# raphiniert-com/volume_renderer

Hardware: AMD Instinct MI355X
Metric: Mrays/s + achieved HBM GB/s, 1024³ vol @ 1920×1080 HG-shaded, 1/2/4/8 GPU (higher is better)
Workload: dtype f32; 1 GPU; V_shell(1024) fp32 1024^3, 1920x1080, HG 2 lights (example1.m), on-the-fly gradient, rotate(125,25,0) f=3 dist=6 thr=0.9; lights=2, gradient=compute, parallelism=image-column partition x1 (block 16), depth_lanes=2, frames=serial, one HIP stream

## Files before the change

include/vrhip.h:

```cpp
#ifndef VRHIP_H_
#define VRHIP_H_

#include <stddef.h>
#include <stdint.h>

#ifdef __cplusplus
extern "C" {
#endif

enum vr_status {
  VR_OK = 0,
  VR_ERR_ARGUMENT = 1,
  VR_ERR_HANDLE = 2,
  VR_ERR_VRAM = 3,
  VR_ERR_DEVICE = 4,
  VR_ERR_UNSUPPORTED = 5
};

enum vr_location { VR_HOST = 0, VR_DEVICE = 1 };

enum vr_dtype { VR_F32 = 0, VR_U8 = 1, VR_U16 = 2, VR_I16 = 3, VR_F16 = 4 };
#define VR_DTYPE_UNORM 0x100

typedef struct vr_volume {
// ... 95 lines not shown
int vr_render_isosurface_device(vr_context *h, const vr_render_args *args, float level, const vr_partition *part,
                                float *d_out, float *d_depth, float *d_normal,
                                unsigned long long *d_steps , void *stream);

int64_t vr_partition_columns(int64_t w, const vr_partition *part);

int vr_assemble_partitions(const float *d_parts, int64_t w, int64_t h, int32_t block_cols,
                           int32_t num_parts, int64_t max_cols, float *d_out, void *stream);

#define VR_SLAB_PLANES 10
typedef struct vr_slab {
  uint64_t depth;
  uint64_t z_first;
  double z0, z1;
  int32_t direction;
  int32_t reserved;
} vr_slab;
int vr_render_slab(vr_context *h, const vr_render_args *args, const vr_slab *slab, const vr_partition *part,
                   const float *d_state_in, float *d_state_out, void *stream);

int vr_slab_planes(const uint64_t dims[3], const float element_size_um[3], double z0, double z1, uint64_t *first,
                   uint64_t *count);

int vr_depth_lanes(int64_t part_cols, int64_t height);
int vr_depth_lanes_tau(int64_t part_cols, int64_t height, double texels_per_pixel);

int vr_synth_shell_device(float *d_out, uint64_t n, void *stream);

int vr_synth_shell_planes_device(float *d_out, uint64_t n, uint64_t z_first, uint64_t count, void *stream);

int vr_gradient_device(const float *d_data, const uint64_t dims[3], float *d_gx, float *d_gy, float *d_gz,
                       void *stream);


int vr_henyey_greenstein_device(uint32_t n, float g, float *d_out, void *stream);

int vr_normalize_device(const float *d_in, uint64_t n, double new_min, double new_max, float *d_out, void *stream);

int vr_resize_device(const float *d_in, const uint64_t in_dims[3], const uint64_t out_dims[3], float *d_out,
                     void *stream);

int vr_resize_contributions(uint64_t in_len, uint64_t out_len, int32_t *P, double *w, int32_t *idx);

int vr_debug_slot_transition(const int32_t idx_in[3], int32_t sim_em_ab, int32_t sim_em_re,
                             int32_t sim_ab_re, int32_t req_em, int32_t req_ab, int32_t req_re,
                             int32_t idx_out[3], int32_t unbound_out[3]);

const char *vr_last_error(void);

int64_t vr_hip_errors(char *buf, size_t buflen);

int vr_last_march_kernel(char *buf, size_t buflen);

int vr_set_option(const char *name, int64_t value);

const char *vr_version(void);

#ifdef __cplusplus
}
#endif
#endif
```

volume_renderer_amd/_lib.py:

```python
from __future__ import annotations

import ctypes
import os
from ctypes import POINTER, c_char_p, c_float, c_int, c_int32, c_int64, c_size_t, c_uint32, c_uint64, c_void_p

_HERE = os.path.dirname(os.path.abspath(__file__))
_DEFAULT_PATH = os.path.join(_HERE, "libvrhip.so")
LIB_PATH = os.environ.get("VR_LIB_PATH") or _DEFAULT_PATH

VR_OK = 0
VR_HOST = 0
VR_DEVICE = 1
VR_F32, VR_U8, VR_U16, VR_I16, VR_F16 = 0, 1, 2, 3, 4
VR_DTYPE_UNORM = 0x100
VR_PROJ_MIP, VR_PROJ_SUM = 0, 1


class VrVolume(ctypes.Structure):
    _fields_ = [("data", c_void_p), ("dims", c_uint64 * 3), ("last_update", c_uint64),
                ("location", c_int32), ("dtype", c_int32)]


class VrLight(ctypes.Structure):
    _fields_ = [("position", c_float * 3), ("color", c_float * 3)]
# ... 30 lines not shown
        super().__init__(msg)
        self.code = code


_lib = None

SIGNATURES = [
    ("vr_new", c_int, [POINTER(c_void_p)]),
    ("vr_new_multi", c_int, [POINTER(c_int32), c_int32, POINTER(c_void_p)]),
    ("vr_delete", c_int, [c_void_p]),
    ("vr_mem_info", c_int, [c_void_p, c_char_p, c_size_t]),
    ("vr_sync_volumes", c_int, [c_void_p, c_uint64, POINTER(VrVolume), POINTER(VrVolume), POINTER(VrVolume),
                                POINTER(VrVolume), POINTER(VrVolume), POINTER(VrVolume)]),
    ("vr_render", c_int, [c_void_p, POINTER(VrRenderArgs), c_void_p]),
    ("vr_render_stereo", c_int, [c_void_p, POINTER(VrRenderArgs), c_float, c_void_p, c_void_p]),
    ("vr_render_channels", c_int, [POINTER(VrChannel), c_int32, c_int32, c_float, c_void_p]),
    ("vr_render_channels_device", c_int, [POINTER(VrChannel), c_int32, c_int32, c_float, c_void_p, c_void_p]),
    ("vr_sum_channels_device", c_int, [c_void_p, c_int32, c_int32, c_uint64, c_void_p, c_void_p]),
    ("vr_henyey_greenstein", c_int, [c_uint32, c_float, c_void_p]),
    ("vr_timestamp", c_uint64, []),
    ("vr_dtype_size", c_size_t, [c_int32]),
    ("vr_convert_host", c_int, [c_void_p, c_int32, c_uint64, c_void_p]),
    ("vr_render_device", c_int, [c_void_p, POINTER(VrRenderArgs), POINTER(VrPartition), c_void_p, c_void_p,
                                 c_void_p]),
    ("vr_render_stereo_device", c_int, [c_void_p, POINTER(VrRenderArgs), c_float, c_void_p, c_void_p, c_void_p,
                                        c_void_p]),
    ("vr_render_projection", c_int, [c_void_p, POINTER(VrRenderArgs), c_int32, c_void_p, c_void_p]),
    ("vr_render_projection_device", c_int, [c_void_p, POINTER(VrRenderArgs), c_int32, POINTER(VrPartition), c_void_p,
                                            c_void_p, c_void_p, c_void_p]),
    ("vr_render_isosurface", c_int, [c_void_p, POINTER(VrRenderArgs), c_float, c_void_p, c_void_p, c_void_p]),
    ("vr_render_isosurface_device", c_int, [c_void_p, POINTER(VrRenderArgs), c_float, POINTER(VrPartition), c_void_p,
                                            c_void_p, c_void_p, c_void_p, c_void_p]),
    ("vr_partition_columns", c_int64, [c_int64, POINTER(VrPartition)]),
    ("vr_assemble_partitions", c_int, [c_void_p, c_int64, c_int64, c_int32, c_int32, c_int64, c_void_p,
                                       c_void_p]),
    ("vr_depth_lanes", c_int, [c_int64, c_int64]),
    ("vr_depth_lanes_tau", c_int, [c_int64, c_int64, ctypes.c_double]),
    ("vr_render_slab", c_int, [c_void_p, POINTER(VrRenderArgs), POINTER(VrSlab), POINTER(VrPartition), c_void_p,
                                c_void_p, c_void_p]),
    ("vr_slab_planes", c_int, [POINTER(c_uint64), POINTER(c_float), ctypes.c_double, ctypes.c_double,
                               POINTER(c_uint64), POINTER(c_uint64)]),
    ("vr_synth_shell_device", c_int, [c_void_p, c_uint64, c_void_p]),
    ("vr_synth_shell_planes_device", c_int, [c_void_p, c_uint64, c_uint64, c_uint64, c_void_p]),
    ("vr_gradient_device", c_int, [c_void_p, POINTER(c_uint64), c_void_p, c_void_p, c_void_p, c_void_p]),
    ("vr_henyey_greenstein_device", c_int, [c_uint32, c_float, c_void_p, c_void_p]),
    ("vr_normalize_device", c_int, [c_void_p, c_uint64, ctypes.c_double, ctypes.c_double, c_void_p, c_void_p]),
    ("vr_resize_device", c_int, [c_void_p, POINTER(c_uint64), POINTER(c_uint64), c_void_p, c_void_p]),
    ("vr_resize_contributions", c_int, [c_uint64, c_uint64, POINTER(c_int32), c_void_p, c_void_p]),
    ("vr_debug_slot_transition", c_int, [POINTER(c_int32), c_int32, c_int32, c_int32, c_int32, c_int32, c_int32,
                                         POINTER(c_int32), POINTER(c_int32)]),
    ("vr_last_error", c_char_p, []),
    ("vr_hip_errors", c_int64, [c_char_p, c_size_t]),
    ("vr_last_march_kernel", c_int, [c_char_p, c_size_t]),
    ("vr_set_option", c_int, [c_char_p, c_int64]),
    ("vr_version", c_char_p, []),
]


def lib():
    global _lib
    if _lib is None:
        try:
            import torch
        except Exception:
            pass
        if not os.path.exists(LIB_PATH):
            raise ImportError(f"libvrhip.so not built at {LIB_PATH}: run __graft_entry__.build() "
                              "(make -C volume_renderer_amd/csrc)")
        handle = ctypes.CDLL(LIB_PATH)
        for name, res, args in SIGNATURES:
            if LIB_PATH != _DEFAULT_PATH and not hasattr(handle, name):
                continue
            fn = getattr(handle, name)
            fn.restype = res
            fn.argtypes = args
        _lib = handle
    return _lib


def check(rc: int) -> None:
    if rc != VR_OK:
        msg = lib().vr_last_error().decode(errors="replace")
        raise VrError(rc, msg)


def hip_errors() -> tuple[int, list[str]]:
    buf = ctypes.create_string_buffer(32 * 400)
    n = lib().vr_hip_errors(buf, len(buf))
    return int(n), [l for l in buf.value.decode(errors="replace").splitlines() if l]
```

volume_renderer_amd/csrc/vr_capi.hip:

```cpp
#include <hip/hip_runtime.h>

#include <algorithm>
#include <chrono>
#include <cmath>
#include <cstdio>
#include <cstdlib>
#include <cstring>
#include <memory>
#include <mutex>
#include <map>
#include <set>
#include <array>
#include <sstream>
#include <string>
#include <queue>
#include <vector>

#include "../../include/vrhip.h"
#include "vr_device.h"
#include "vr_resources.h"

#ifndef VR_WITH_K8
#define VR_WITH_K8 0
#endif
// ... 824 lines not shown
    slots = cus * 16;
  }
  return slots;
}

#ifndef VR_COUNT_K
#define VR_COUNT_K 0
#endif
#ifndef VR_XCD_RUN
#define VR_XCD_RUN 0
#endif

int depth_lanes(const vr::RenderParams &P) {
  if (const char *ev = test_env("VR_DEPTH_LANES")) {
    const int k = std::atoi(ev);
    if (k == 1 || k == 2 || k == 4 || (k == 8 && VR_WITH_K8)) return k;
  }
  const double waves = std::ceil(P.part_cols / 8.0) * std::ceil(P.height / 8.0);
  const double rounds = waves / device_wave_slots();
  const double tau = P.tau > 0.f ? (double)P.tau : 1.0;
  if (P.lookup) return 4;
  if (rounds < VR_DEPTH_ROUNDS_K2 || tau >= VR_DEPTH_TAU_K4) return 4;
  if (rounds >= VR_DEPTH_ROUNDS_K1 && tau < VR_DEPTH_TAU_K1) return 1;
  return 2;
}

void set_tau_and_slot(vr::RenderParams &P, const vr_render_args *a, double vw) {
  const double f = std::fabs((double)a->props[1]), dist = std::fabs((double)a->props[2]);
  const double tau = (f > 0 && P.width > 0) ? dist * vw / ((double)P.width * f) : 1e30;
  P.tau = (float)std::min(tau, 1e30);
  const int K = P.steps ? 1 : depth_lanes(P);
  P.wide_slot = (tau > 1.5 || (K >= 4 && !P.lookup)) ? 1 : 0;
  if (const char *ev = test_env("VR_WIDE_SLOT")) P.wide_slot = std::atoi(ev) ? 1 : 0;
}

bool short_launch(const vr::RenderParams &P) {
  const double rounds = std::ceil(P.part_cols / 8.0) * std::ceil(P.height / 8.0) * std::max(1, (int)P.views) /
                        device_wave_slots();
  return rounds < VR_SCHED_ROUNDS;
}
#ifndef VR_SCHED_LPT_ROUNDS
#define VR_SCHED_LPT_ROUNDS 32.0
#endif
bool lpt_launch(const vr::RenderParams &P) {
  const double rounds = std::ceil(P.part_cols / 8.0) * std::ceil(P.height / 8.0) * std::max(1, (int)P.views) /
                        device_wave_slots();
  return rounds < VR_SCHED_ROUNDS || rounds >= VR_SCHED_LPT_ROUNDS;
}
bool want_schedule(const vr::RenderParams &P) {
  if (P.views > 2 || (P.views == 2 && test_flag("VR_STEREO_PAIR")) || test_flag_off("VR_SCHED")) return false;
  return test_flag("VR_SCHED") || short_launch(P) || !test_flag_off("VR_SCHED_FULL");
}

uint64_t wg_tail_arg(uint32_t tail_pct) {
  return (uint64_t)tail_pct << 32 | (uint64_t)(device_wave_slots() / 16 * 6);
}

uint64_t frame_key(const vr::RenderParams &P) {
  uint64_t h = 1469598103934665603ull;
  auto mix = [&h](const void *p, size_t n) {
    const unsigned char *c = static_cast<const unsigned char *>(p);
    for (size_t i = 0; i < n; ++i) h = (h ^ c[i]) * 1099511628211ull;
  };
  mix(P.eye, sizeof P.eye);
  mix(P.eye2, sizeof P.eye2);
  mix(P.nx_, sizeof P.nx_);
  mix(P.ydir, sizeof P.ydir);
  mix(P.zdir, sizeof P.zdir);
  mix(&P.focal, sizeof P.focal);
  mix(P.bmin, sizeof P.bmin);
  mix(&P.tstep, sizeof P.tstep);
  mix(&P.thr, sizeof P.thr);
  mix(&P.fa, sizeof P.fa);
  mix(&P.fe, sizeof P.fe);
  mix(&P.em.p, sizeof P.em.p);
  mix(&P.occ, sizeof P.occ);
  const BufPtr &eb = g_tex.bind[g_tex.idx_em];
  const uint64_t ver = (eb && eb->ptr == P.em.p) ? eb->version : 0;
  mix(&ver, sizeof ver);
  return h | 1u;
}

#ifndef VR_PRED_STEP_TEXELS
#define VR_PRED_STEP_TEXELS 8.0
#endif
hipError_t predict_costs(const vr::RenderParams &P, int K, uint32_t nb_view, uint32_t *cost, hipStream_t stream) {
  const int TW = K == 1 ? 8 : (K == 2 ? 4 : (K == 4 ? 4 : 2)), TH = K <= 2 ? 8 : 4;
  const uint32_t nbx = (uint32_t)((P.part_cols + 2 * TW - 1) / (2 * TW));
  const BufPtr &eb = g_tex.bind[g_tex.idx_em];
  double dens = 0.0;
  if (eb && !eb->nonfinite && P.fa > 0.f && std::isfinite(P.fa))
    dens = (double)P.fa * (double)eb->maxabs / 255.0 * (double)P.tstep;
  const double xthr = P.thr < 1.f ? -std::log1p(-(double)std::max(P.thr, 0.f)) : 1e30;
  double tpa = 0.0;
  for (int i = 0; i < 3; ++i) {
    const float n = i == 0 ? P.em.fnx : (i == 1 ? P.em.fny : P.em.fnz);
    tpa = std::max(tpa, (double)P.bscale[i] * (double)n);
  }
  const double per = (double)P.tstep * tpa;
  const int m = (int)std::max(1.0, std::min(4096.0, std::floor(VR_PRED_STEP_TEXELS / std::max(per, 1e-9))));
  const hipError_t rc = vr::launch_predict_cost(P, nb_view, nbx, TW, TH, m, (float)dens, (float)std::min(xthr, 1e30),
                                                cost, stream);
  if (const char *dump = rc == hipSuccess ? diag_env("VR_SCHED_PRED_DUMP") : nullptr) {
    const uint32_t nb = nb_view * (uint32_t)std::max(1, (int)P.views);
    std::vector<uint32_t> c(nb);
    VR_HIP(hipMemcpyAsync(c.data(), cost, (size_t)nb * 4, hipMemcpyDeviceToHost, stream));
    VR_HIP(hipStreamSynchronize(stream));
    const uint32_t hdr[4] = {(uint32_t)K, (uint32_t)P.part, (uint32_t)P.num_parts, nb};
    if (FILE *f = std::fopen(dump, "ab")) {
// ... 30 lines not shown
    S.blocks = nb;
  }
  if (!(S.d_cost && S.blocks == nb)) return hipSuccess;
  hipError_t rc = hipSuccess;
  const bool full = !lpt_launch(P) && !test_flag("VR_SCHED");
  const uint64_t fkey = frame_key(P);
  const bool predict = P.occ && P.occ_bx && !diag_flag("VR_SCHED_MEASURED");
  if (!full) {
    P.sched_full = 0;
    if (S.measured && S.key == fkey) {
      rc = vr::launch_order(S.d_cost, nb, S.d_order, stream, 0u, 0u);
    } else if (predict) {
      rc = predict_costs(P, K, nb_view, S.d_cost, stream);
      if (rc == hipSuccess) rc = vr::launch_order(S.d_cost, nb, S.d_order, stream, 0u, 0u);
    } else {
      rc = vr::launch_iota(S.d_order, nb, stream);
    }
    S.measured = true;
    S.key = fkey;
    S.pred_key = 0;
  } else {
    if (S.key != fkey) {
      if (S.copy_pending) {
        (void)hipEventSynchronize(S.copied);
        S.copy_pending = false;
      }
      S.measured = S.decided = S.tail = S.order_stale = false;
      S.frames = S.renders = 0;
      S.key = fkey;
    }
    ++S.renders;
    uint32_t every = VR_SCHED_REMEASURE;
    if (const char *ev = test_env("VR_SCHED_REMEASURE")) every = (uint32_t)std::max(1, std::atoi(ev));
    uint32_t heavy_div = VR_SCHED_HEAVY_DIV;
    if (const char *ev = diag_env("VR_SCHED_HEAVY_DIV")) heavy_div = (uint32_t)std::max(1, std::atoi(ev));
    uint32_t tail_pct = VR_SCHED_TAIL_PCT;
    if (const char *ev = test_env("VR_SCHED_TAIL_PCT")) tail_pct = (uint32_t)std::max(0, std::atoi(ev));
    if (!S.h_cost) {
      hipError_t e = hipHostMalloc(reinterpret_cast<void **>(&S.h_cost), nb * sizeof(uint32_t));
      if (e == hipSuccess) e = hipEventCreateWithFlags(&S.copied, hipEventDisableTiming);
      if (e != hipSuccess) {
        vr_host::consume(e, "hipHostMalloc / hipEventCreate (full-frame schedule; none used)");
        return hipSuccess;
      }
    }
    if (S.copy_pending && vr_host::query_done(S.copied, "hipEventQuery (schedule durations)")) {
      S.copy_pending = false;
      uint64_t sum = 0;
      uint32_t mx = 0;
      for (uint32_t i = 0; i < nb; ++i) {
        sum += S.h_cost[i];
        mx = std::max(mx, S.h_cost[i]);
      }
      const uint64_t wg_slots = std::max<uint64_t>(1, (uint64_t)(device_wave_slots() / 16 * 6));
      S.tail = (uint64_t)mx * 100u >= (sum / wg_slots) * tail_pct;
      S.decided = true;
      S.order_stale = true;
    }
    if (predict && !S.decided) {
      if (S.pred_key != fkey) {
        rc = predict_costs(P, K, nb_view, S.d_cost, stream);
        if (rc == hipSuccess) rc = vr::launch_order(S.d_cost, nb, S.d_order, stream, heavy_div, wg_tail_arg(0));
        S.pred_key = rc == hipSuccess ? fkey : 0;
      }
      if (S.renders >= 2 && !S.measured && !diag_flag("VR_SCHED_PREDICT_ONLY")) {
        S.measured = true;
        S.frames = 0;
        P.sched_full = 1;
        F.sched_copy = &S;
      } else {
        P.sched_full = 2;
      }
    } else {
      S.pred_key = 0;
      bool measure = !S.measured;
      if (S.measured && !S.copy_pending && ++S.frames >= every) measure = true;
      if (measure) {
        S.frames = 0;
        if (S.decided && S.tail) {
          if (S.order_stale) rc = vr::launch_order(S.d_cost, nb, S.d_order, stream, heavy_div, wg_tail_arg(0));
        } else {
          rc = vr::launch_iota(S.d_order, nb, stream);
        }
        S.order_stale = false;
        S.measured = true;
        P.sched_full = 1;
        F.sched_copy = &S;
      } else if (S.decided && S.tail) {
        if (S.order_stale) {
          rc = vr::launch_order(S.d_cost, nb, S.d_order, stream, heavy_div, wg_tail_arg(0));
          S.order_stale = false;
        }
        P.sched_full = 2;
      } else {
        return hipSuccess;
      }
    }
  }
  if (rc != hipSuccess) return rc;
  P.wg_order = S.d_order;
  P.wg_cost = S.d_cost;
  P.sched_blocks = nb;
  P.prio_blocks = P.sched_full ? 0u : (uint32_t)(device_wave_slots() / 4);
  if (const char *ev = diag_env("VR_PRIO_BLOCKS")) P.prio_blocks = (uint32_t)std::atoi(ev);
  return hipSuccess;
}

void time_mark(vr_context *h, int which, hipStream_t stream) {
// ... 89 lines not shown
        vr_host::consume(ea, "pooled_alloc (interleaved lookup gradient; three separate gathers instead)");
        gv->ptr = nullptr;
      }
    }
    if (G.buf) {
      P.gvec = G.buf->ptr;
      P.gv_row8 = 8u * ((gpx + 1) >> 1);
      P.gv_plane8 = P.gv_row8 * ((gpy + 1) >> 1);
    }
  }
  if (fusable && march && F.mode <= 1 && !F.big && !P.steps) {
    *fusable = 1;
    return VR_OK;
  }
  LaunchRec L;
  L.stream = stream;
  L.device = h->device;
  bind_reads(L);
  stage_frame(L, P, g_tex.lights);
  if (march) {
    const int K = (P.steps && !(VR_COUNT_K && test_flag("VR_COUNT_PROD"))) ? 1
                                                                          : exact_lanes(depth_lanes(P), P.fast_shade);
    set_chunk_halo(F, K);
    typedef hipError_t (*launch_fn)(const vr::RenderParams &, int, bool, bool, bool, hipStream_t);
    typedef uint32_t (*blocks_fn)(const vr::RenderParams &);
    static const launch_fn fns[2][4] = {
        {vr::exact::launch_march_k1, vr::exact::launch_march_k2,
         VR_EXACT_K4(vr::exact::launch_march_k4, vr::exact::launch_march_k2),
         VR_K8(vr::exact::launch_march_k8, vr::exact::launch_march_k2)},
        {vr::fast::launch_march_k1, vr::fast::launch_march_k2, vr::fast::launch_march_k4,
         VR_K8(vr::fast::launch_march_k8, vr::fast::launch_march_k4)}};
    const int ki = K == 1 ? 0 : K == 2 ? 1 : K == 4 ? 2 : 3;
    if (!P.steps && K > 1 && P.fast_shade && F.ab_alias && want_schedule(P))
      VR_HIP(attach_schedule(h, P, F, K, stream, ""));
    if (P.views > 1) {
      static const blocks_fn vfns[4] = {vr::fast::march_blocks_k1, vr::fast::march_blocks_k2,
                                        vr::fast::march_blocks_k4,
                                        VR_K8(vr::fast::march_blocks_k8, vr::fast::march_blocks_k4)};
      P.view_blocks = vfns[ki](P);
      if (test_flag("VR_STEREO_PAIR") && K > 1 && P.fast_shade && F.mode == 1 && F.ab_alias && P.tap_half &&
          !P.wide_slot && !F.big && P.num_parts == 1 && !P.wg_order) {
        const double base = std::fabs((double)a->props[0]), f = std::fabs((double)a->props[1]),
                     dist = std::fabs((double)a->props[2]);
        const int TW = 4;
        const double cols = dist > 0 ? base * (double)P.width * f / dist : 0.0;
        P.pair_shift = (int32_t)std::min<double>(std::floor(cols / TW + 0.5) * TW, (double)P.width);
        if (const char *ev = test_env("VR_STEREO_PAIR_SHIFT")) P.pair_shift = std::max(0, std::atoi(ev));
      }
    }
    const char *dump = (P.wg_cost && P.sched_full != 2) ? test_env("VR_SCHED_DUMP") : nullptr;
    uint32_t *d_start = nullptr;
    if (dump) {
      const hipError_t e = hipMalloc(reinterpret_cast<void **>(&d_start), (size_t)P.sched_blocks * 4);
      if (e == hipSuccess) P.wg_start = d_start;
      else vr_host::consume(e, "hipMalloc (VR_SCHED_DUMP start ticks; not recorded)");
    }
    if (const char *ev = test_env("VR_BLOCK_ROT_ROWS")) {
      const int TW = K == 1 ? 8 : (K == 2 ? 4 : (K == 4 ? 4 : 2));
      const uint32_t nbx = (uint32_t)((P.part_cols + 2 * TW - 1) / (2 * TW));
      typedef uint32_t (*bfn)(const vr::RenderParams &);
      static const bfn bf[4] = {vr::fast::march_blocks_k1, vr::fast::march_blocks_k2, vr::fast::march_blocks_k4,
                                VR_K8(vr::fast::march_blocks_k8, vr::fast::march_blocks_k4)};
      const uint32_t nb = bf[ki](P) * (P.views > 1 ? 2u : 1u);
      const uint64_t rot = (uint64_t)std::max(0, std::atoi(ev)) * nbx;
      P.block_rot = nb ? (uint32_t)(rot % nb) : 0u;
    }
    if (VR_PRELEAP_LAUNCH && F.sched && F.sched->blocks && P.occ && P.tame && !P.pair_shift && P.fast_shade &&
        !test_flag("VR_NO_PRELEAP")) {
      vr_context::Schedule &S = *F.sched;
      const uint32_t waves = S.blocks * (uint32_t)VR_WG_WAVES_HOST;
      if (S.pre_waves != waves) {
        if (S.pre_flag) (void)hipFree(S.pre_flag);
        if (S.pre_state) (void)hipFree(S.pre_state);
        S.pre_flag = nullptr;
        S.pre_state = nullptr;
        S.pre_waves = S.pre_cap = 0;
        const uint32_t cap = std::max<uint32_t>(64u, waves / 8u);
        hipError_t e = S.pre_count ? hipSuccess : hipMalloc(reinterpret_cast<void **>(&S.pre_count), 4);
        if (e == hipSuccess) e = hipMalloc(reinterpret_cast<void **>(&S.pre_flag), (size_t)waves * 4);
        if (e == hipSuccess) e = hipMalloc(reinterpret_cast<void **>(&S.pre_state), (size_t)cap * 64 * 2 * sizeof(float4));
        if (e == hipSuccess) {
          S.pre_waves = waves;
          S.pre_cap = cap;
        } else {
          vr_host::consume(e, "hipMalloc (pre-leap buffers; the launch marches without)");
        }
      }
      if (S.pre_waves == waves) {
        P.pre_flag = S.pre_flag;
        P.pre_state = S.pre_state;
        P.pre_count = S.pre_count;
        P.pre_cap = S.pre_cap;
        typedef hipError_t (*pre_fn)(const vr::RenderParams &, hipStream_t);
        static const pre_fn pfns[4] = {vr::fast::launch_preleap_k1, vr::fast::launch_preleap_k2,
                                       vr::fast::launch_preleap_k4,
                                       VR_K8(vr::fast::launch_preleap_k8, vr::fast::launch_preleap_k4)};
        VR_HIP(hipMemsetAsync(S.pre_count, 0, 4, stream));
        VR_HIP(pfns[ki](P, stream));
      }
    }
    time_mark(h, 0, stream);
    {
      const hipError_t e = fns[P.fast_shade ? 1 : 0][ki](P, F.mode, F.ab_alias, F.share, F.big, stream);
      if (e != hipSuccess) throw HipError{e, "the march kernel launch (launch_march_k)"};
    }
    time_mark(h, 1, stream);
    if (F.sched_copy) {
      vr_context::Schedule &S = *F.sched_copy;
      VR_HIP(hipMemcpyAsync(S.h_cost, S.d_cost, (size_t)S.blocks * sizeof(uint32_t), hipMemcpyDeviceToHost, stream));
      VR_HIP(hipEventRecord(S.copied, stream));
      S.copy_pending = true;
      F.sched_copy = nullptr;
    }
    if (dump) {
      std::vector<uint32_t> c(P.sched_blocks), st(d_start ? P.sched_blocks : 0);
      VR_HIP(hipMemcpyAsync(c.data(), P.wg_cost, c.size() * 4, hipMemcpyDeviceToHost, stream));
      if (d_start) VR_HIP(hipMemcpyAsync(st.data(), d_start, st.size() * 4, hipMemcpyDeviceToHost, stream));
      VR_HIP(hipStreamSynchronize(stream));
      if (d_start) (void)hipFree(d_start);
      const uint32_t hdr[4] = {(uint32_t)K, (uint32_t)P.part, (uint32_t)P.num_parts, P.sched_blocks};
      if (FILE *f = std::fopen(dump, "ab")) {
        std::fwrite(hdr, 4, 4, f);
        std::fwrite(c.data(), 4, c.size(), f);
        std::fclose(f);
      }
      if (d_start)
        if (FILE *f = std::fopen((std::string(dump) + ".start").c_str(), "ab")) {
          std::fwrite(hdr, 4, 4, f);
          std::fwrite(st.data(), 4, st.size(), f);
          std::fclose(f);
        }
    }
  } else {
    VR_HIP(vr::launch_render(P, F.mode, F.ab_alias, F.big, F.share, stream));
    if (P.views > 1) {
      for (int i = 0; i < 3; ++i) P.eye[i] = P.eye2[i];
      P.out = P.out2;
      VR_HIP(vr::launch_render(P, F.mode, F.ab_alias, F.big, F.share, stream));
    }
  }
  VR_HIP(L.finish());
  return VR_OK;
}

int do_project(vr_context *h, const vr_render_args *a, int32_t mode, const vr_partition *part, float *d_out,
               float *d_aux, unsigned long long *d_steps, hipStream_t stream) {
  Frame F;
  int rc = build_frame(h, a, F);
  if (rc) return rc;
  rc = validate_partition(part);
  if (rc) return rc;
  vr::RenderParams &P = F.P;
  P.block_cols = part ? part->block_cols : std::max<int32_t>(P.width, 1);
// ... 1375 lines not shown
  switch (dtype) {
    case VR_F32: convert_host<float, false>(src, n, dst); break;
    case VR_U8: convert_host<uint8_t, false>(src, n, dst); break;
    case VR_U8 | VR_DTYPE_UNORM: convert_host<uint8_t, true>(src, n, dst); break;
    case VR_U16: convert_host<uint16_t, false>(src, n, dst); break;
    case VR_U16 | VR_DTYPE_UNORM: convert_host<uint16_t, true>(src, n, dst); break;
    case VR_I16: convert_host<int16_t, false>(src, n, dst); break;
    case VR_F16: convert_host<vr::half_bits, false>(src, n, dst); break;
  }
  return VR_OK;
}

uint64_t vr_timestamp(void) {
  const auto ms = std::chrono::duration_cast<std::chrono::milliseconds>(
                      std::chrono::system_clock::now().time_since_epoch())
                      .count();
  return (uint64_t)(uint32_t)(uint64_t)ms;
}

const char *vr_last_error(void) { return g_last_error.c_str(); }

int64_t vr_hip_errors(char *buf, size_t buflen) {
  vr_host::ErrLog &L = vr_host::errlog();
  std::lock_guard<std::mutex> g(L.mu);
  if (buf && buflen) {
    std::string s;
    for (const std::string &l : L.lines) s += l + "\n";
    const size_t n = std::min(buflen - 1, s.size());
    std::memcpy(buf, s.data(), n);
    buf[n] = 0;
  }
  return (int64_t)L.count;
}

int vr_set_option(const char *name, int64_t value) {
  if (name && std::strcmp(name, "test_switches") == 0) {
    g_test_switches.store(value ? 1 : 0);
    return VR_OK;
  }
  return fail(VR_ERR_ARGUMENT, std::string("unknown option ") + (name ? name : "(null)"));
}

int vr_last_march_kernel(char *buf, size_t buflen) {
  std::lock_guard<std::mutex> lk(g_mu);
  const std::string &s = vr::last_march_kernel();
  if (buf && buflen) {
    const size_t n = std::min(buflen - 1, s.size());
    std::memcpy(buf, s.data(), n);
    buf[n] = 0;
  }
  return VR_OK;
}

const char *vr_version(void) { return "libvrhip 0.1 gfx950 (MI355X) volume ray-marcher"; }

}
```

volume_renderer_amd/csrc/vr_device.h:

```cpp
#pragma once
#include <stdint.h>
#include <hip/hip_runtime.h>

namespace vr {

struct DevTex {
  const float *p;
  int32_t nx, ny, nz;
  uint32_t px;
  uint32_t pxy;
  float fnx, fny, fnz;
  int32_t one;
  int32_t small;
  float fpx4, fpxy4, fbase4;
  const float *zp;
};

#ifndef VR_PROBE_MAX
#define VR_PROBE_MAX 512
#endif

#ifndef VR_OCC_LOG
#define VR_OCC_LOG 3
#endif
// ... 26 lines not shown
  float tap_off[3];
  int32_t tap_half;
  float cube_hs[3];
  int32_t num_lights;
  const DevLight *lights;
  DevTex em, ab, re, gem, gx, gy, gz, lut;
  const float *gvec;
  uint32_t gv_row8, gv_plane8;
  int32_t re_is_em;
  int32_t skip_empty;
  int32_t small_x;
  int32_t eds_finite;
  int32_t tame;
  uint32_t re_mask;
  float tau;
  int32_t lookup;
  int32_t tile_mode;
  int32_t xcd_run;
  uint32_t block_rot;
  int32_t wide_slot;
  int32_t fast_shade;
  int32_t block_cols, part, num_parts, part_cols;
  int32_t plane_cols;
  float *out;
  float *out2;
  int32_t views;
  int32_t pair_shift;
  uint32_t view_blocks;
  const uint32_t *wg_order;
  uint32_t *wg_cost;
  uint32_t *wg_start;
  uint32_t sched_blocks;
  uint32_t sched_full;
  uint32_t prio_blocks;
  const uint8_t *occ;
  uint32_t occ_bx, occ_bxy;
  float probe_off[3];
  unsigned long long *steps;
  float slab_z0, slab_z1, slab_margin;
  int32_t slab_pk0, slab_pk1, slab_dir;
  const float *slab_in;
  const uint32_t *pre_flag;
  float4 *pre_state;
  uint32_t *pre_count;
  uint32_t pre_cap;
};

#define VR_VIEWS_MAX 4
struct RenderViews {
  RenderParams p[VR_VIEWS_MAX];
};
static_assert(sizeof(RenderViews) <= 4160, "RenderParams grew: RenderViews passes four by value as kernel arguments");

struct BufStats {
  uint32_t nonfinite;
  float maxabs;
};

void note_march_kernel(bool fast, int K, int mode, bool ab, bool count, bool share, bool big, int cap, int sched,
                       int nl);
bool test_switches_on();

}
```

volume_renderer_amd/csrc/vr_march.hip:

```cpp
#include <hip/hip_runtime.h>
#include <stdint.h>
#include <math.h>
#include <stdlib.h>
#include <algorithm>
#include <type_traits>

#ifndef VR_MARCH_K
#define VR_MARCH_K 1
#endif
#ifndef VR_MERGED_BOUNDS
#define VR_MERGED_BOUNDS 1
#endif
#ifndef VR_WHOLE_BOX
#define VR_WHOLE_BOX 1
#endif
#ifndef VR_CHECK_WHOLE
#define VR_CHECK_WHOLE 0
#endif
#ifndef VR_LIGHTS_HOIST
#define VR_LIGHTS_HOIST 1
#endif
#ifndef VR_REFL_HOIST
#define VR_REFL_HOIST 1
#endif
// ... 563 lines not shown
                                                         R.o, r, gg, b, alpha, shaded, rv, pre);
        }
        if (COUNT) {
          ++C.iter;
          C.lit += (MODE != 0 && __any(shaded)) ? 1u : 0u;
        }
        composite_group<K, 0, VR_ZERO_FILL && !NANCHK && !SLAB>(P, R, ex ? 1.f : 0.f, r, gg, b, alpha, thr);
        if (SLAB && !inside) {
          if (R.alive && group_any<K>(R.mine && !ex)) {
            float t = R.t;
            f3 p = R.pos;
            int32_t n = R.nsteps;
            first_of_group<K>((R.mine && !ex) ? 1.f : 0.f, R.t, R.pos, R.nsteps, t, p, n);
            if (sub == 0) store_resume(P, kk, t, p, n);
            R.alive = false;
            R.past = true;
          }
        }
        if constexpr (!NANCHK && !SLAB)
          advance_k<K>(P, R.mine, R.nsteps, R.t, R.tfar, R.pos, R.step, cap);
        else
          advance(P, K, R.mine, R.nsteps, R.t, R.tfar, R.pos, R.step, cap);
        R.alive = R.alive && group_any<K>(R.mine);
      }
      };
      if constexpr (VR_WHOLE_SPLIT && !NANCHK && !SLAB && VR_MARCH_FAST && MODE == 1 && SHARE2) {
        if (whole) samples(std::true_type{});
        else samples(std::false_type{});
      } else {
        samples(std::false_type{});
      }
    }
    unpark();
    __builtin_amdgcn_wave_barrier();
  }
}

__device__ __forceinline__ bool finite3(const f3 &v) {
  return fabsf(v.x) <= 3.4e38f && fabsf(v.y) <= 3.4e38f && fabsf(v.z) <= 3.4e38f;
}

#ifndef VR_MARCH_MIN_EU
#define VR_MARCH_MIN_EU 5
#endif
#ifndef VR_SCHED1_MIN_EU
#define VR_SCHED1_MIN_EU 1
#endif
constexpr int march_min_eu(int cap, int sched) {
  return cap <= VR_LDS_CAP_MARCH ? (sched != 1 ? VR_MARCH_MIN_EU : VR_SCHED1_MIN_EU) : 1;
}
#ifndef VR_WG_WAVES
#define VR_WG_WAVES 4
#endif

template <int K>
struct TileShape {
  static constexpr int LR = (K == 1 ? 6 : K == 2 ? 5 : K == 4 ? 4 : 3);
  static constexpr int LK = 6 - LR;
#ifndef VR_TILE_WLOG
#define VR_TILE_WLOG -1
#endif
  static constexpr int LW = (VR_TILE_WLOG >= 0 && VR_TILE_WLOG <= LR) ? VR_TILE_WLOG : LR / 2;
  static constexpr int TW = 1 << LW, TH = 1 << (LR - LW);
};

__device__ __forceinline__ uint32_t xcd_block(uint32_t b, uint32_t n, int run) {
  if (run <= 1) return b;
  const uint32_t R = (uint32_t)run, gs = 8u * R, g = b / gs;
  if ((g + 1) * gs > n) return b;
  const uint32_t r = b - g * gs;
  return g * gs + (r & 7u) * R + (r >> 3);
}

template <int K, int MODE, bool AB_ALIAS, bool COUNT, bool SHARE2, bool BIG, int CAP, int SCHED, int NL>
__global__ __launch_bounds__(64 * VR_WG_WAVES, march_min_eu(CAP, SCHED)) void march_kernel(const RenderParams P) {
  using TS = TileShape<K>;
  __shared__ float lds[VR_WG_WAVES][CAP];
  const int lane = threadIdx.x & 63, wave = threadIdx.x >> 6;
  float *L = lds[wave];
  constexpr bool ORDERED = SCHED >= 1 && SCHED <= 3;
  constexpr bool TIMED = SCHED == 1 || SCHED == 2;
  constexpr bool PAIRED = SCHED == 4;
  const uint64_t clk0 = TIMED ? __builtin_amdgcn_s_memrealtime() : 0;
  uint32_t wgo = ORDERED ? P.wg_order[blockIdx.x] : xcd_block(blockIdx.x, gridDim.x, P.xcd_run);
  if (!ORDERED && P.block_rot) {
    wgo += P.block_rot;
    if (wgo >= gridDim.x) wgo -= gridDim.x;
  }
  if (ORDERED && blockIdx.x < P.prio_blocks) __builtin_amdgcn_s_setprio(2);
  int view, lc, y;
  if constexpr (PAIRED) {
    constexpr int TH2 = TS::TH / 2, HR = (64 / K) / 2;
    const int tile = (int)wgo * VR_WG_WAVES + wave;
    const int nbx = (P.part_cols + P.pair_shift + 2 * TS::TW - 1) / (2 * TS::TW);
    const int blk = tile >> 2, quad = tile & 3;
    const int ray = lane >> TS::LK, rr = ray & (HR - 1);
    view = ray >= HR ? 0 : 1;
    const int xv = (blk % nbx) * (2 * TS::TW) + (quad & 1) * TS::TW + rr / TH2;
    y = (blk / nbx) * (2 * TH2) + (quad >> 1) * TH2 + rr % TH2;
    lc = view ? xv - P.pair_shift : xv;
  } else {
    view = (P.views > 1 && wgo >= P.view_blocks) ? 1 : 0;
    const uint32_t wg = view ? wgo - P.view_blocks : wgo;
    const int tile = (int)wg * VR_WG_WAVES + wave;
    const int nbx = (P.part_cols + 2 * TS::TW - 1) / (2 * TS::TW);
    const int blk = tile >> 2, quad = tile & 3;
    const int ray = lane >> TS::LK;
    lc = (blk % nbx) * (2 * TS::TW) + (quad & 1) * TS::TW + (ray / TS::TH);
    y = (blk / nbx) * (2 * TS::TH) + (quad >> 1) * TS::TH + (ray % TS::TH);
  }
  float *const out = view ? P.out2 : P.out;
  const bool active = (!PAIRED || lc >= 0) && (lc < P.part_cols) && (y < P.height);
  Ray R;
  R.o = mk(0.f, 0.f, 0.f);
  R.pos = R.o;
  R.step = R.o;
  R.t = 0.f;
  R.tfar = -1.f;
  R.sr = R.sg = R.sb = R.sa = 0.f;
  R.nsteps = R.nlit = 0;
  R.alive = false;
  ChunkStats C{0, 0, 0, 0, 0, 0, 0};
  if (active) {
    const int blk = lc / P.block_cols, within = lc - blk * P.block_cols;
    const int x = (P.part + blk * P.num_parts) * P.block_cols + within;
    f3 d;
    float tnear;
    R.alive = ray_setup(P, x, y, R.o, d, tnear, R.tfar, view);
    R.pos = mk(fmaf(d.x, tnear, R.o.x), fmaf(d.y, tnear, R.o.y), fmaf(d.z, tnear, R.o.z));
    R.step = mk(d.x * P.tstep, d.y * P.tstep, d.z * P.tstep);
    R.t = tnear;
  }
  if (P.tame && __all(!R.alive || (finite3(R.pos) && finite3(R.step))))
    march<K, MODE, AB_ALIAS, COUNT, SHARE2, BIG, false, CAP, false, NL>(
        P, L, lane, R, C, 0u, (KParams)__builtin_amdgcn_kernarg_segment_ptr(), wgo * VR_WG_WAVES + (uint32_t)wave);
  else
    march<K, MODE, AB_ALIAS, COUNT, SHARE2, BIG, true, CAP>(P, L, lane, R, C);

  if (active && (lane & (K - 1)) == 0) {
    const size_t plane = (size_t)P.plane_cols * (size_t)P.height;
    const size_t kk = (size_t)lc * (size_t)P.height + (size_t)y;
    out[kk] = R.sr;
    out[kk + plane] = R.sg;
    out[kk + 2 * plane] = R.sb;
  }
  if (TIMED) {
    __syncthreads();
    if (threadIdx.x == 0) {
      const uint64_t d = __builtin_amdgcn_s_memrealtime() - clk0;
      P.wg_cost[wgo] = d > 0xffffffffull ? 0xffffffffu : (uint32_t)d;
      if (P.wg_start) P.wg_start[wgo] = (uint32_t)clk0;
    }
  }
  if (COUNT) {
    unsigned long long s = K == 1 ? (unsigned long long)R.nsteps : 0ull, l = K == 1 ? (unsigned long long)R.nlit : 0ull;
#pragma unroll
    for (int off = 32; off > 0; off >>= 1) {
      s += __shfl_xor(s, off, 64);
      l += __shfl_xor(l, off, 64);
    }
    if (lane == 0 && s) atomicAdd(P.steps, s);
    if (lane == 0 && l) atomicAdd(P.steps + 1, l);
    if (lane == 0) {
      atomicAdd(P.steps + 2, (unsigned long long)C.staged);
      atomicAdd(P.steps + 3, (unsigned long long)C.leap);
      atomicAdd(P.steps + 4, (unsigned long long)C.fall);
      atomicAdd(P.steps + 5, (unsigned long long)C.iter);
      atomicAdd(P.steps + 6, (unsigned long long)C.lit);
      atomicAdd(P.steps + 7, (unsigned long long)C.probe);
      atomicAdd(P.steps + 44, (unsigned long long)C.probe_fail);
    }
  }
}

template <int K>
__global__ __launch_bounds__(64 * VR_WG_WAVES) void preleap_kernel(const RenderParams P) {
  using TS = TileShape<K>;
  const int lane = threadIdx.x & 63, wave = threadIdx.x >> 6;
  const uint32_t wgo = blockIdx.x;
  const uint32_t gw = wgo * VR_WG_WAVES + (uint32_t)wave;
  const int view = (P.views > 1 && wgo >= P.view_blocks) ? 1 : 0;
  const uint32_t wg = view ? wgo - P.view_blocks : wgo;
  const int tile = (int)wg * VR_WG_WAVES + wave;
  const int nbx = (P.part_cols + 2 * TS::TW - 1) / (2 * TS::TW);
  const int blk = tile >> 2, quad = tile & 3;
  const int ray = lane >> TS::LK;
  const int lc = (blk % nbx) * (2 * TS::TW) + (quad & 1) * TS::TW + (ray / TS::TH);
  const int y = (blk / nbx) * (2 * TS::TH) + (quad >> 1) * TS::TH + (ray % TS::TH);
  const bool active = lc < P.part_cols && y < P.height;
  Ray R;
  R.pos = mk(0.f, 0.f, 0.f);
  R.step = R.pos;
  R.t = 0.f;
  R.tfar = -1.f;
  R.nsteps = 0;
  R.alive = false;
  if (active) {
    const int pb = lc / P.block_cols, within = lc - pb * P.block_cols;
    const int x = (P.part + pb * P.num_parts) * P.block_cols + within;
    f3 o, d;
    float tnear;
    R.alive = ray_setup(P, x, y, o, d, tnear, R.tfar, view);
    R.pos = mk(fmaf(d.x, tnear, o.x), fmaf(d.y, tnear, o.y), fmaf(d.z, tnear, o.z));
    R.step = mk(d.x * P.tstep, d.y * P.tstep, d.z * P.tstep);
// ... 251 lines not shown
}

#if !VR_ISA_PROBE
template <int MODE, bool SH, int CAP>
static void launch_slab_c(const RenderParams &P, dim3 grid, hipStream_t s) {
  constexpr int K = VR_MARCH_K;
  const dim3 blk(64 * VR_WG_WAVES);
  if (P.wg_order) hipLaunchKernelGGL((march_slab_kernel<K, MODE, SH, CAP, true>), grid, blk, 0, s, P);
  else hipLaunchKernelGGL((march_slab_kernel<K, MODE, SH, CAP, false>), grid, blk, 0, s, P);
}

template <int MODE, bool SH>
static void launch_slab_m(const RenderParams &P, dim3 grid, hipStream_t s) {
  if (P.wide_slot) launch_slab_c<MODE, SH, VR_LDS_CAP_WIDE>(P, grid, s);
  else launch_slab_c<MODE, SH, VR_LDS_CAP>(P, grid, s);
}

hipError_t VR_CAT(launch_march_slab_k, VR_MARCH_K)(const RenderParams &P, int mode, hipStream_t s) {
  constexpr int K = VR_MARCH_K;
  using TS = TileShape<K>;
  if (P.part_cols <= 0 || P.height <= 0) return hipSuccess;
  if (mode > 1) return hipErrorInvalidValue;
  const uint64_t tiles = (uint64_t)((P.part_cols + 2 * TS::TW - 1) / (2 * TS::TW)) *
                         (uint64_t)((P.height + 2 * TS::TH - 1) / (2 * TS::TH)) * 4;
  const dim3 grid((unsigned)((tiles + VR_WG_WAVES - 1) / VR_WG_WAVES));
  if (P.wg_order && (P.sched_blocks != grid.x || !P.wg_cost || K == 1)) return hipErrorInvalidValue;
  if (mode == 0) launch_slab_m<0, false>(P, grid, s);
  else if (VR_MARCH_FAST && P.tap_half) launch_slab_m<1, true>(P, grid, s);
  else launch_slab_m<1, false>(P, grid, s);
  return hipGetLastError();
}
#endif
#endif

#if !VR_ISA_PROBE
static bool inject_bad_launch() {
  const char *ev = test_switches_on() ? getenv("VR_INJECT_BAD_LAUNCH") : nullptr;
  return ev && ev[0] == '1';
}

template <int KK, int MODE, bool AB, bool CNT, bool SH, bool BG, int CAP, int SC>
static void launch_one(const RenderParams &P, dim3 grid, dim3 blk, hipStream_t s) {
  constexpr bool NL2 = VR_NL2 && VR_LIGHTS_HOIST && MODE == 1 && KK > 1 && AB && SH && !BG && !CNT;
  const int nl = (NL2 && (P.num_lights == 2 || P.num_lights == 1)) ? P.num_lights : 0;
  if (NL2 && nl == 2) hipLaunchKernelGGL((march_kernel<KK, MODE, AB, CNT, SH, BG, CAP, SC, NL2 ? 2 : 0>), grid, blk, 0, s, P);
  else if (NL2 && nl == 1) hipLaunchKernelGGL((march_kernel<KK, MODE, AB, CNT, SH, BG, CAP, SC, NL2 ? 1 : 0>), grid, blk, 0, s, P);
  else hipLaunchKernelGGL((march_kernel<KK, MODE, AB, CNT, SH, BG, CAP, SC, 0>), grid, blk, 0, s, P);
  note_march_kernel(VR_MARCH_FAST, KK, MODE, AB, CNT, SH, BG, CAP, SC, nl);
}

template <int MODE, bool AB, bool SH, int CAP, int BS = 3>
static hipError_t launch_c(const RenderParams &P, dim3 grid, hipStream_t s, bool big) {
  constexpr int K = VR_MARCH_K;
  const dim3 blk(inject_bad_launch() ? 2048 : 64 * VR_WG_WAVES);
  const bool sched = P.wg_order && P.wg_cost;
  constexpr bool SCH = K > 1 && VR_MARCH_FAST && AB;
  constexpr int S1 = SCH ? 1 : 0, S2 = SCH ? 2 : 0, S3 = SCH ? 3 : 0;
#define VR_LAUNCH(KK, CNT, BG, SC) launch_one<KK, MODE, AB, CNT, SH, BG, CAP, SC>(P, grid, blk, s)
#define VR_LAUNCH_B(KK, CNT, SC)                                                                           \
  do {                                                                                                    \
    if (big) {                                                                                            \
      if constexpr ((BS & 2) != 0) VR_LAUNCH(KK, CNT, true, SC);                                          \
      else return hipErrorInvalidValue;                                                                   \
    } else {                                                                                              \
      if constexpr ((BS & 1) != 0) VR_LAUNCH(KK, CNT, false, SC);                                         \
      else return hipErrorInvalidValue;                                                                   \
    }                                                                                                     \
  } while (0)
  constexpr bool PAIRK = K > 1 && VR_MARCH_FAST && AB && MODE == 1 && SH && CAP == VR_LDS_CAP_MARCH && (BS & 1);
  if (P.pair_shift) {
    if constexpr (PAIRK) {
      if (big || sched || (P.steps && !VR_COUNT_K)) return hipErrorInvalidValue;
      if (P.steps) VR_LAUNCH(K, VR_COUNT_K != 0, false, 4);
      else VR_LAUNCH(K, false, false, 4);
      return hipGetLastError();
    } else {
      return hipErrorInvalidValue;
    }
  }
  if constexpr (K == 1 || VR_COUNT_K) {
    if (P.steps) {
      VR_LAUNCH_B(K, true, 0);
      return hipGetLastError();
    }
  }
  if (P.steps) {
    return hipErrorInvalidValue;
  } else if (sched && !SCH) {
    return hipErrorInvalidValue;
  } else if (K > 1 && sched && P.sched_full == 1) {
    VR_LAUNCH_B(K, false, S2);
  } else if (K > 1 && sched && P.sched_full == 2) {
    VR_LAUNCH_B(K, false, S3);
  } else if (K > 1 && sched) {
    VR_LAUNCH_B(K, false, S1);
  } else {
    VR_LAUNCH_B(K, false, 0);
  }
#undef VR_LAUNCH_B
#undef VR_LAUNCH
  return hipGetLastError();
}

template <int MODE, bool AB, bool SH>
static hipError_t launch_m(const RenderParams &P, dim3 grid, hipStream_t s, bool big) {
  if (P.wide_slot) return launch_c<MODE, AB, SH, VR_LDS_CAP_WIDE>(P, grid, s, big);
  if constexpr (MODE == 2 || !VR_MARCH_FAST)
    return launch_c<MODE, AB, SH, VR_LDS_CAP>(P, grid, s, big);
  else
    return big ? launch_c<MODE, AB, SH, VR_LDS_CAP, 2>(P, grid, s, big)
               : launch_c<MODE, AB, SH, VR_LDS_CAP_MARCH, 1>(P, grid, s, big);
}

uint32_t VR_CAT(march_blocks_k, VR_MARCH_K)(const RenderParams &P) {
  using TS = TileShape<VR_MARCH_K>;
  if (P.part_cols <= 0 || P.height <= 0) return 0;
  const uint64_t tiles = (uint64_t)((P.part_cols + 2 * TS::TW - 1) / (2 * TS::TW)) *
                         (uint64_t)((P.height + 2 * TS::TH - 1) / (2 * TS::TH)) * 4;
  return (uint32_t)((tiles + VR_WG_WAVES - 1) / VR_WG_WAVES);
}

hipError_t VR_CAT(launch_march_k, VR_MARCH_K)(const RenderParams &P, int mode, bool ab_alias, bool share, bool big,
                                              hipStream_t s) {
  using TS = TileShape<VR_MARCH_K>;
  if (P.part_cols <= 0 || P.height <= 0) return hipSuccess;
  if (VR_MARCH_K != 1 && !VR_COUNT_K && P.steps) return hipErrorInvalidValue;
  const uint64_t tiles = (uint64_t)((P.part_cols + 2 * TS::TW - 1) / (2 * TS::TW)) *
                         (uint64_t)((P.height + 2 * TS::TH - 1) / (2 * TS::TH)) * 4;
  const uint32_t per_view = (uint32_t)((tiles + VR_WG_WAVES - 1) / VR_WG_WAVES);
  if (P.views > 1 && (P.view_blocks != per_view || !P.out2)) return hipErrorInvalidValue;
  dim3 grid(per_view * (P.views > 1 ? 2u : 1u));
  if (P.pair_shift) {
    if (P.views != 2 || P.num_parts != 1 || P.pair_shift < 0 || P.wg_order) return hipErrorInvalidValue;
    const uint64_t ptiles = (uint64_t)((P.part_cols + P.pair_shift + 2 * TS::TW - 1) / (2 * TS::TW)) *
                            (uint64_t)((P.height + TS::TH - 1) / TS::TH) * 4;
    grid = dim3((unsigned)((ptiles + VR_WG_WAVES - 1) / VR_WG_WAVES));
  }
  if (P.wg_order && (P.sched_blocks != grid.x || !P.wg_cost || VR_MARCH_K == 1))
    return hipErrorInvalidValue;
  switch (mode) {
    case 0: return ab_alias ? launch_m<0, true, false>(P, grid, s, big) : launch_m<0, false, false>(P, grid, s, big);
    case 1:
      if (VR_MARCH_FAST && P.tap_half)
        return ab_alias ? launch_m<1, true, true>(P, grid, s, big) : launch_m<1, false, true>(P, grid, s, big);
      return ab_alias ? launch_m<1, true, false>(P, grid, s, big) : launch_m<1, false, false>(P, grid, s, big);
    default:
      if (share) return ab_alias ? launch_m<2, true, true>(P, grid, s, big) : launch_m<2, false, true>(P, grid, s, big);
      return ab_alias ? launch_m<2, true, false>(P, grid, s, big) : launch_m<2, false, false>(P, grid, s, big);
  }
}

#else
template __global__ void march_kernel<2, 1, true, false, true, false, VR_LDS_CAP_MARCH, 0, 2>(const RenderParams P);
template __global__ void march_kernel<2, 2, true, false, true, false, VR_LDS_CAP, 0, 0>(const RenderParams P);
template __global__ void march_slab_kernel<2, 1, true, VR_LDS_CAP, false>(const RenderParams P);
#endif
}
}
```

Measured before the change: 83.90 Mrays/s.

## Allow march workgroups of 1 or 2 waves with XCD-aware tile dispatch

```diff
diff --git a/include/vrhip.h b/include/vrhip.h
--- a/include/vrhip.h
+++ b/include/vrhip.h
@@ -171,6 +171,11 @@
 
 int vr_last_march_kernel(char *buf, size_t buflen);
 
+int vr_march_wg_waves(void);
+
+int vr_debug_march_dispatch(uint32_t nb, int32_t waves, int32_t xcd_run, uint32_t *slot, uint32_t *block,
+                            uint32_t *quad);
+
 int vr_set_option(const char *name, int64_t value);
 
 const char *vr_version(void);
diff --git a/volume_renderer_amd/_lib.py b/volume_renderer_amd/_lib.py
--- a/volume_renderer_amd/_lib.py
+++ b/volume_renderer_amd/_lib.py
@@ -106,6 +106,9 @@
     ("vr_last_error", c_char_p, []),
     ("vr_hip_errors", c_int64, [c_char_p, c_size_t]),
     ("vr_last_march_kernel", c_int, [c_char_p, c_size_t]),
+    ("vr_march_wg_waves", c_int, []),
+    ("vr_debug_march_dispatch", c_int, [c_uint32, c_int32, c_int32, POINTER(c_uint32), POINTER(c_uint32),
+                                        POINTER(c_uint32)]),
     ("vr_set_option", c_int, [c_char_p, c_int64]),
     ("vr_version", c_char_p, []),
 ]
diff --git a/volume_renderer_amd/csrc/vr_capi.hip b/volume_renderer_amd/csrc/vr_capi.hip
--- a/volume_renderer_amd/csrc/vr_capi.hip
+++ b/volume_renderer_amd/csrc/vr_capi.hip
@@ -900,9 +900,9 @@
   return test_flag("VR_SCHED") || short_launch(P) || !test_flag_off("VR_SCHED_FULL");
 }
 
-uint64_t wg_tail_arg(uint32_t tail_pct) {
-  return (uint64_t)tail_pct << 32 | (uint64_t)(device_wave_slots() / 16 * 6);
-}
+uint64_t resident_blocks() { return std::max<uint64_t>(1, (uint64_t)(device_wave_slots() / 16 * 5)); }
+
+uint64_t wg_tail_arg(uint32_t tail_pct) { return (uint64_t)tail_pct << 32 | resident_blocks(); }
 
 uint64_t frame_key(const vr::RenderParams &P) {
   uint64_t h = 1469598103934665603ull;
@@ -1039,8 +1039,7 @@
         sum += S.h_cost[i];
         mx = std::max(mx, S.h_cost[i]);
       }
-      const uint64_t wg_slots = std::max<uint64_t>(1, (uint64_t)(device_wave_slots() / 16 * 6));
-      S.tail = (uint64_t)mx * 100u >= (sum / wg_slots) * tail_pct;
+      S.tail = (uint64_t)mx * 100u >= (sum / resident_blocks()) * tail_pct;
       S.decided = true;
       S.order_stale = true;
     }
@@ -1236,8 +1235,12 @@
     uint32_t *d_start = nullptr;
     if (dump) {
       const hipError_t e = hipMalloc(reinterpret_cast<void **>(&d_start), (size_t)P.sched_blocks * 4);
-      if (e == hipSuccess) P.wg_start = d_start;
-      else vr_host::consume(e, "hipMalloc (VR_SCHED_DUMP start ticks; not recorded)");
+      if (e == hipSuccess) {
+        VR_HIP(hipMemsetAsync(d_start, 0xff, (size_t)P.sched_blocks * 4, stream));
+        P.wg_start = d_start;
+      } else {
+        vr_host::consume(e, "hipMalloc (VR_SCHED_DUMP start ticks; not recorded)");
+      }
     }
     if (const char *ev = test_env("VR_BLOCK_ROT_ROWS")) {
       const int TW = K == 1 ? 8 : (K == 2 ? 4 : (K == 4 ? 4 : 2));
@@ -1283,6 +1286,8 @@
         VR_HIP(pfns[ki](P, stream));
       }
     }
+    if (VR_MARCH_WG_WAVES < VR_WG_WAVES_HOST && P.wg_cost && P.sched_full != 2)
+      VR_HIP(hipMemsetAsync(P.wg_cost, 0, (size_t)P.sched_blocks * sizeof(uint32_t), stream));
     time_mark(h, 0, stream);
     {
       const hipError_t e = fns[P.fast_shade ? 1 : 0][ki](P, F.mode, F.ab_alias, F.share, F.big, stream);
@@ -2764,6 +2769,24 @@
   return VR_OK;
 }
 
+int vr_march_wg_waves(void) { return VR_MARCH_WG_WAVES; }
+
+int vr_debug_march_dispatch(uint32_t nb, int32_t waves, int32_t xcd_run, uint32_t *slot, uint32_t *block,
+                            uint32_t *quad) {
+  if (waves == 0) waves = VR_MARCH_WG_WAVES;
+  if ((waves != 1 && waves != 2 && waves != 4) || !slot || !block || !quad)
+    return fail(VR_ERR_ARGUMENT, "vr_debug_march_dispatch: waves in {0, 1, 2, 4} and three output arrays");
+  const uint64_t n = (uint64_t)nb * (uint64_t)(4 / waves);
+  if (n > 0x7fffffffull) return fail(VR_ERR_ARGUMENT, "vr_debug_march_dispatch: more workgroups than a launch holds");
+  for (uint32_t b = 0; b < (uint32_t)n; ++b) {
+    const vr::MarchSlot ms = vr::march_dispatch(b, nb, waves);
+    slot[b] = ms.slot;
+    block[b] = vr::xcd_block(ms.slot, nb, xcd_run);
+    quad[b] = ms.quad;
+  }
+  return VR_OK;
+}
+
 const char *vr_version(void) { return "libvrhip 0.1 gfx950 (MI355X) volume ray-marcher"; }
 
 }
diff --git a/volume_renderer_amd/csrc/vr_device.h b/volume_renderer_amd/csrc/vr_device.h
--- a/volume_renderer_amd/csrc/vr_device.h
+++ b/volume_renderer_amd/csrc/vr_device.h
@@ -102,6 +102,32 @@
 };
 static_assert(sizeof(RenderViews) <= 4160, "RenderParams grew: RenderViews passes four by value as kernel arguments");
 
+#ifndef VR_MARCH_WG_WAVES
+#define VR_MARCH_WG_WAVES 4
+#endif
+static_assert(VR_MARCH_WG_WAVES == 1 || VR_MARCH_WG_WAVES == 2 || VR_MARCH_WG_WAVES == 4,
+              "march workgroups of 1, 2 or 4 waves");
+
+__host__ __device__ __forceinline__ uint32_t xcd_block(uint32_t b, uint32_t n, int run) {
+  if (run <= 1) return b;
+  const uint32_t R = (uint32_t)run, gs = 8u * R, g = b / gs;
+  if ((g + 1) * gs > n) return b;
+  const uint32_t r = b - g * gs;
+  return g * gs + (r & 7u) * R + (r >> 3);
+}
+
+struct MarchSlot {
+  uint32_t slot, quad;
+};
+__host__ __device__ __forceinline__ MarchSlot march_dispatch(uint32_t b, uint32_t nb, int waves) {
+  if (waves >= 4) return MarchSlot{b, 0u};
+  const uint32_t per = 4u / (uint32_t)waves, gs = 8u * per;
+  const uint32_t g = b / gs, r = b - g * gs;
+  if (8u * (g + 1u) <= nb) return MarchSlot{8u * g + (r & 7u), (r >> 3) * (uint32_t)waves};
+  const uint32_t m = nb - 8u * g;
+  return MarchSlot{8u * g + r % m, (r / m) * (uint32_t)waves};
+}
+
 struct BufStats {
   uint32_t nonfinite;
   float maxabs;
diff --git a/volume_renderer_amd/csrc/vr_march.hip b/volume_renderer_amd/csrc/vr_march.hip
--- a/volume_renderer_amd/csrc/vr_march.hip
+++ b/volume_renderer_amd/csrc/vr_march.hip
@@ -639,6 +639,7 @@
 #ifndef VR_WG_WAVES
 #define VR_WG_WAVES 4
 #endif
+static_assert(VR_WG_WAVES == 4, "a block is 2x2 tiles (march_dispatch, the schedules, the pre-leap slots)");
 
 template <int K>
 struct TileShape {
@@ -651,34 +652,29 @@
   static constexpr int TW = 1 << LW, TH = 1 << (LR - LW);
 };
 
-__device__ __forceinline__ uint32_t xcd_block(uint32_t b, uint32_t n, int run) {
-  if (run <= 1) return b;
-  const uint32_t R = (uint32_t)run, gs = 8u * R, g = b / gs;
-  if ((g + 1) * gs > n) return b;
-  const uint32_t r = b - g * gs;
-  return g * gs + (r & 7u) * R + (r >> 3);
-}
-
 template <int K, int MODE, bool AB_ALIAS, bool COUNT, bool SHARE2, bool BIG, int CAP, int SCHED, int NL>
-__global__ __launch_bounds__(64 * VR_WG_WAVES, march_min_eu(CAP, SCHED)) void march_kernel(const RenderParams P) {
+__global__ __launch_bounds__(64 * VR_MARCH_WG_WAVES, march_min_eu(CAP, SCHED)) void march_kernel(const RenderParams P) {
   using TS = TileShape<K>;
-  __shared__ float lds[VR_WG_WAVES][CAP];
+  __shared__ float lds[VR_MARCH_WG_WAVES][CAP];
   const int lane = threadIdx.x & 63, wave = threadIdx.x >> 6;
   float *L = lds[wave];
   constexpr bool ORDERED = SCHED >= 1 && SCHED <= 3;
   constexpr bool TIMED = SCHED == 1 || SCHED == 2;
   constexpr bool PAIRED = SCHED == 4;
   const uint64_t clk0 = TIMED ? __builtin_amdgcn_s_memrealtime() : 0;
-  uint32_t wgo = ORDERED ? P.wg_order[blockIdx.x] : xcd_block(blockIdx.x, gridDim.x, P.xcd_run);
+  const uint32_t nb = gridDim.x / (VR_WG_WAVES / VR_MARCH_WG_WAVES);
+  const MarchSlot ms = march_dispatch(blockIdx.x, nb, VR_MARCH_WG_WAVES);
+  const int twave = (int)ms.quad + wave;
+  uint32_t wgo = ORDERED ? P.wg_order[ms.slot] : xcd_block(ms.slot, nb, P.xcd_run);
   if (!ORDERED && P.block_rot) {
     wgo += P.block_rot;
-    if (wgo >= gridDim.x) wgo -= gridDim.x;
-  }
-  if (ORDERED && blockIdx.x < P.prio_blocks) __builtin_amdgcn_s_setprio(2);
+    if (wgo >= nb) wgo -= nb;
+  }
+  if (ORDERED && ms.slot < P.prio_blocks) __builtin_amdgcn_s_setprio(2);
   int view, lc, y;
   if constexpr (PAIRED) {
     constexpr int TH2 = TS::TH / 2, HR = (64 / K) / 2;
-    const int tile = (int)wgo * VR_WG_WAVES + wave;
+    const int tile = (int)wgo * VR_WG_WAVES + twave;
     const int nbx = (P.part_cols + P.pair_shift + 2 * TS::TW - 1) / (2 * TS::TW);
     const int blk = tile >> 2, quad = tile & 3;
     const int ray = lane >> TS::LK, rr = ray & (HR - 1);
@@ -689,7 +685,7 @@
   } else {
     view = (P.views > 1 && wgo >= P.view_blocks) ? 1 : 0;
     const uint32_t wg = view ? wgo - P.view_blocks : wgo;
-    const int tile = (int)wg * VR_WG_WAVES + wave;
+    const int tile = (int)wg * VR_WG_WAVES + twave;
     const int nbx = (P.part_cols + 2 * TS::TW - 1) / (2 * TS::TW);
     const int blk = tile >> 2, quad = tile & 3;
     const int ray = lane >> TS::LK;
@@ -720,7 +716,7 @@
   }
   if (P.tame && __all(!R.alive || (finite3(R.pos) && finite3(R.step))))
     march<K, MODE, AB_ALIAS, COUNT, SHARE2, BIG, false, CAP, false, NL>(
-        P, L, lane, R, C, 0u, (KParams)__builtin_amdgcn_kernarg_segment_ptr(), wgo * VR_WG_WAVES + (uint32_t)wave);
+        P, L, lane, R, C, 0u, (KParams)__builtin_amdgcn_kernarg_segment_ptr(), wgo * VR_WG_WAVES + (uint32_t)twave);
   else
     march<K, MODE, AB_ALIAS, COUNT, SHARE2, BIG, true, CAP>(P, L, lane, R, C);
 
@@ -731,12 +727,18 @@
     out[kk + plane] = R.sg;
     out[kk + 2 * plane] = R.sb;
   }
-  if (TIMED) {
+  if constexpr (TIMED && VR_MARCH_WG_WAVES == VR_WG_WAVES) {
     __syncthreads();
     if (threadIdx.x == 0) {
       const uint64_t d = __builtin_amdgcn_s_memrealtime() - clk0;
       P.wg_cost[wgo] = d > 0xffffffffull ? 0xffffffffu : (uint32_t)d;
       if (P.wg_start) P.wg_start[wgo] = (uint32_t)clk0;
+    }
+  } else if constexpr (TIMED) {
+    if (lane == 0) {
+      const uint64_t d = __builtin_amdgcn_s_memrealtime() - clk0;
+      atomicMax(&P.wg_cost[wgo], d > 0xffffffffull ? 0xffffffffu : (uint32_t)d);
+      if (P.wg_start) atomicMin(&P.wg_start[wgo], (uint32_t)clk0);
     }
   }
   if (COUNT) {
@@ -1094,7 +1096,7 @@
 template <int MODE, bool AB, bool SH, int CAP, int BS = 3>
 static hipError_t launch_c(const RenderParams &P, dim3 grid, hipStream_t s, bool big) {
   constexpr int K = VR_MARCH_K;
-  const dim3 blk(inject_bad_launch() ? 2048 : 64 * VR_WG_WAVES);
+  const dim3 blk(inject_bad_launch() ? 2048 : 64 * VR_MARCH_WG_WAVES);
   const bool sched = P.wg_order && P.wg_cost;
   constexpr bool SCH = K > 1 && VR_MARCH_FAST && AB;
   constexpr int S1 = SCH ? 1 : 0, S2 = SCH ? 2 : 0, S3 = SCH ? 3 : 0;
@@ -1171,15 +1173,17 @@
                          (uint64_t)((P.height + 2 * TS::TH - 1) / (2 * TS::TH)) * 4;
   const uint32_t per_view = (uint32_t)((tiles + VR_WG_WAVES - 1) / VR_WG_WAVES);
   if (P.views > 1 && (P.view_blocks != per_view || !P.out2)) return hipErrorInvalidValue;
-  dim3 grid(per_view * (P.views > 1 ? 2u : 1u));
+  uint64_t blocks = (uint64_t)per_view * (P.views > 1 ? 2u : 1u);
   if (P.pair_shift) {
     if (P.views != 2 || P.num_parts != 1 || P.pair_shift < 0 || P.wg_order) return hipErrorInvalidValue;
     const uint64_t ptiles = (uint64_t)((P.part_cols + P.pair_shift + 2 * TS::TW - 1) / (2 * TS::TW)) *
                             (uint64_t)((P.height + TS::TH - 1) / TS::TH) * 4;
-    grid = dim3((unsigned)((ptiles + VR_WG_WAVES - 1) / VR_WG_WAVES));
-  }
-  if (P.wg_order && (P.sched_blocks != grid.x || !P.wg_cost || VR_MARCH_K == 1))
+    blocks = (ptiles + VR_WG_WAVES - 1) / VR_WG_WAVES;
+  }
+  if (P.wg_order && (P.sched_blocks != blocks || !P.wg_cost || VR_MARCH_K == 1))
     return hipErrorInvalidValue;
+  if (blocks * (VR_WG_WAVES / VR_MARCH_WG_WAVES) > 0x7fffffffull) return hipErrorInvalidValue;
+  const dim3 grid((unsigned)(blocks * (VR_WG_WAVES / VR_MARCH_WG_WAVES)));
   switch (mode) {
     case 0: return ab_alias ? launch_m<0, true, false>(P, grid, s, big) : launch_m<0, false, false>(P, grid, s, big);
     case 1:
```

After: 83.67 Mrays/s. About the same (-0.3%).
